# Luoyadan/CRB-active-3Ddet

Measured on AMD Instinct MI355X. Metric: frames/s SECOND fwd+bwd, KITTI 20k-pt clouds, higher is better.
Workload: dtype f32

## Files before the change

### crb-active-3ddet_amd/pcdet/models/backbones_2d/base_bev_backbone.py

```python
import numpy as np
import torch
import torch.nn as nn

from crbhip import bnrelu

from ...utils.fold_utils import fold_conv_bn
from ...utils.linear_rows import LinearRows, rows_view, rows_to_nchw


ROWS_TRAIN = True
ROWS_GEMM = True
WINOGRAD = __import__('os').environ.get('CRB_WINOGRAD', '1') != '0'


def _wino_fold(w, shift):
    from crbhip import winograd
    return winograd.weights_forward2(w), shift.contiguous()


def _wino_ok(conv, x, pad=None):
    if not WINOGRAD or not isinstance(conv, nn.Conv2d) or not x.is_cuda or x.dtype != torch.float32:
        return False
    from crbhip import winograd
    p = tuple(conv.padding) if pad is None else tuple(pad)
# ... 66 lines not shown
                if rows_ok:
                    y = m(x) if pad is None else torch.nn.functional.conv2d(x, m.weight, None, m.stride, pad, m.dilation,
                                                                             m.groups)
                    rows_ok = y.is_contiguous(memory_format=torch.channels_last) and \
                        bnrelu.supported(y.new_empty((2, y.shape[1])), bn)
                if rows_ok:
                    n, c, h, w_ = y.shape
                    rows = y.permute(0, 2, 3, 1).reshape(n * h * w_, c)
                    z = bnrelu.bn_apply_(rows, bn, relu)
                    x = z.view(n, h, w_, c).permute(0, 3, 1, 2)
                else:
                    w, shift = fold_conv_bn(m, bn)
                    if isinstance(m, nn.Conv2d):
                        x = torch.nn.functional.conv2d(x, w, shift, m.stride, m.padding if pad is None else pad, m.dilation,
                                                       m.groups)
                    else:
                        x = torch.nn.functional.conv_transpose2d(x, w, shift, m.stride, m.padding, m.output_padding,
                                                                 m.groups, m.dilation)
                    if relu:
                        x = torch.relu_(x)
                i += 3 if relu else 2
            else:
                x = m(x) if pad is None else torch.nn.functional.conv2d(x, m.weight, m.bias, m.stride, pad, m.dilation, m.groups)
                i += 1
        return x

    @staticmethod
    def _pad_conv(mods, i, x):
        m = mods[i]
        if isinstance(m, nn.ZeroPad2d) and i + 1 < len(mods) and isinstance(mods[i + 1], nn.Conv2d):
            c = mods[i + 1]
            pd = m.padding
            if c.padding == (0, 0) and c.padding_mode == 'zeros' and pd[0] == pd[1] and pd[2] == pd[3]:
                if _wino_ok(c, x, (pd[2], pd[0])):
                    from crbhip import winograd
                    return BaseBEVBackbone._wino_conv(c, x, mods[i + 2] if i + 2 < len(mods) else None), 2
                if torch.are_deterministic_algorithms_enabled() and torch.is_grad_enabled() and pd[0] == pd[2] and x.is_cuda:
                    from crbhip import dense_strided
                    if dense_strided.supported(c, x):
                        return dense_strided.conv_det(c, x, (pd[2], pd[0])), 2
                return torch.nn.functional.conv2d(x, c.weight, c.bias, c.stride, (pd[2], pd[0]), c.dilation, c.groups), 2
        return None, 0

    @staticmethod
    def _wino_conv(conv, x, nxt):
        from crbhip import winograd
        if winograd.STATS and conv.bias is None and isinstance(nxt, nn.BatchNorm2d) and nxt.training and \
                nxt.momentum is not None and bnrelu.FUSE_RUNNING and torch.is_grad_enabled() and not bnrelu.frame_groups_active():
            y, slabs = winograd.conv3x3_stats(x, conv.weight)
            y._crb_bn_slabs = slabs
            return y
        return winograd.conv3x3(x, conv.weight, conv.bias)

    @staticmethod
    def _run_rows_train(seq, x):
        mods = list(seq)
        i = 0
        while i < len(mods):
            m = mods[i]
            nxt = mods[i + 1] if i + 1 < len(mods) else None
            y, used = BaseBEVBackbone._pad_conv(mods, i, x)
            if used:
                x, i = y, i + used
                continue
            if _wino_ok(m, x):
                x = BaseBEVBackbone._wino_conv(m, x, nxt)
                i += 1
                continue
            if isinstance(m, nn.BatchNorm2d) and isinstance(nxt, nn.ReLU) and \
                    x.is_contiguous(memory_format=torch.channels_last) and \
                    bnrelu.supported(x.new_empty((2, x.shape[1])), m):
                n, c, h, w_ = x.shape
                rows = x.permute(0, 2, 3, 1).reshape(n * h * w_, c)
                slabs = getattr(x, '_crb_bn_slabs', None)
                x = bnrelu.bn_relu(rows, m, relu=True, slabs=slabs).view(n, h, w_, c).permute(0, 3, 1, 2)
                i += 2
            else:
                x = m(x)
                i += 1
        return x

    @staticmethod
    def _up(conv, x):
        if ROWS_GEMM and x.is_cuda and conv.bias is None and conv.kernel_size == (1, 1) and conv.stride == (1, 1) and \
                conv.padding == (0, 0) and conv.groups == 1 and conv.dilation == (1, 1):
            rows = rows_view(x)
            if rows is not None:
                w2d = conv.weight[:, :, 0, 0]
                w2d = w2d.t() if isinstance(conv, nn.ConvTranspose2d) else w2d
                n, _, h, w_ = x.shape
                return rows_to_nchw(LinearRows.apply(rows, w2d), n, h, w_)
        if torch.are_deterministic_algorithms_enabled() and torch.is_grad_enabled() and x.is_cuda and isinstance(conv, nn.ConvTranspose2d):
            from crbhip import dense_strided
            if dense_strided.supported(conv, x):
                return dense_strided.conv_det(conv, x)
        return conv(x)

    def _can_fuse_concat_eval(self, x):
        if len(self.deblocks) != len(self.blocks) or len(self.deblocks) < 2:
            return False
        for d in self.deblocks:
            m = list(d)
            if len(m) != 3 or not isinstance(m[1], nn.BatchNorm2d) or not isinstance(m[2], nn.ReLU) or m[0].bias is not None \
                    or not bnrelu.supported(x.new_empty((2, m[1].num_features)), m[1]):
                return False
        return True

    def _can_fuse_concat(self, x):
        if not self.training or len(self.deblocks) != len(self.blocks) or len(self.deblocks) < 2:
            return False
        for d in self.deblocks:
            m = list(d)
            if len(m) != 3 or not isinstance(m[1], nn.BatchNorm2d) or not isinstance(m[2], nn.ReLU) or \
                    not m[1].training or m[1].momentum is None or \
                    not bnrelu.supported(x.new_empty((2, m[1].num_features)), m[1]):
                return False
        return x.is_contiguous(memory_format=torch.channels_last)

    def forward(self, data_dict):
        spatial_features = data_dict['spatial_features']
        ups = []
        x = spatial_features
        if not self.training and not torch.is_grad_enabled():
            cat_ok = x.is_cuda and x.is_contiguous(memory_format=torch.channels_last) and self._can_fuse_concat_eval(x)
            pre = []
            for i, blk in enumerate(self.blocks):
                x = self._run_folded(blk, x)
                if cat_ok:
                    pre.append(self._up(self.deblocks[i][0], x))
                else:
                    ups.append(self._run_folded(self.deblocks[i], x) if len(self.deblocks) > 0 else x)
            if cat_ok and all(p.is_contiguous(memory_format=torch.channels_last) and p.shape[2:] == pre[0].shape[2:]
                              for p in pre):
                n, _, h, w_ = pre[0].shape
                cat = torch.empty((n * h * w_, sum(p.shape[1] for p in pre)), dtype=torch.float32, device=x.device)
                col = 0
                for d, p in zip(self.deblocks, pre):
                    bnrelu.bn_apply_into(p.permute(0, 2, 3, 1).reshape(n * h * w_, p.shape[1]), d[1], True, cat, col)
                    col += p.shape[1]
                ups = [cat.view(n, h, w_, cat.shape[1]).permute(0, 3, 1, 2)]
            elif cat_ok:
                ups = [self._run_folded(nn.Sequential(*list(d)[1:]), p) for d, p in zip(self.deblocks, pre)]
            x = torch.cat(ups, dim=1) if len(ups) > 1 else ups[0]
            if len(self.deblocks) > len(self.blocks):
                x = self._run_folded(self.deblocks[-1], x)
            data_dict['spatial_features_2d'] = x
            return data_dict
        run = self._run_rows_train if (ROWS_TRAIN and x.is_cuda and x.is_contiguous(memory_format=torch.channels_last)) \
            else (lambda seq, t: seq(t))
        if run == self._run_rows_train and torch.is_grad_enabled():
            from crbhip import winograd
            if winograd.PREPARE:
                winograd.prepare_weights2([m.weight for blk in self.blocks for m in blk
                                           if isinstance(m, nn.Conv2d) and m.kernel_size == (3, 3) and m.stride == (1, 1)
                                           and m.weight.is_cuda])
        fuse_cat = ROWS_TRAIN and x.is_cuda and self._can_fuse_concat(x)
        pre = []
        for i, blk in enumerate(self.blocks):
            x = run(blk, x)
            stride = int(spatial_features.shape[2] / x.shape[2])
            data_dict['spatial_features_%dx' % stride] = x
            if fuse_cat:
                pre.append(self._up(self.deblocks[i][0], x))
            else:
                ups.append(run(self.deblocks[i], x) if len(self.deblocks) > 0 else x)
        if fuse_cat and all(p.is_contiguous(memory_format=torch.channels_last) and p.shape[2:] == pre[0].shape[2:]
# ... 16 lines not shown
```

### include/crb_hip.h

```cpp
#ifndef CRB_HIP_H
#define CRB_HIP_H
#include <stdint.h>

#ifdef __cplusplus
extern "C" {
#endif

#define CRB_OK 0
#define CRB_ERR_ARG (-1)
#define CRB_ERR_WORKSPACE (-2)
#define CRB_ERR_LAUNCH (-3)
#define CRB_ERR_UNSUPPORTED (-4)

int crb_abi_version(void);

int64_t crb_voxelize_workspace_bytes(int64_t n_points, int B, int max_voxels, int max_points);
int crb_voxelize(const float* points, int64_t n_points, int num_features,
                 const int32_t* frame_offsets, int B,
                 const float* range_min_xyz, const float* voxel_size_xyz, const int32_t* grid_xyz,
                 int max_voxels, int max_points,
                 float* voxels, int32_t* coords, int32_t* num_points, float* mean_features,
                 int32_t* num_voxels_out,
                 void* workspace, int64_t workspace_bytes, void* stream);

// ... 308 lines not shown
                         float loss_weight, float* loss, float* d_preds, void* stream);
int crb_point_focal_loss_per_frame(const float* preds, const int64_t* labels, int64_t n, int num_class, int B, float alpha, float gamma,
                                   float loss_weight, float* loss, float* d_preds, void* stream);

typedef struct CrbRcnnLossCfg {
  float beta;
  float code_weights[7];
  float cls_weight, reg_weight, corner_weight;
  int32_t corner;
} CrbRcnnLossCfg;
int crb_rcnn_loss(const float* rcnn_cls, const float* rcnn_reg, const void* cls_labels, int labels_are_int64,
                  const int64_t* reg_valid_mask, const float* rois, const float* gt_of_rois, const float* gt_of_rois_src,
                  int gt_row_stride, int64_t n, const CrbRcnnLossCfg* cfg, float* loss, float* d_cls, float* d_reg,
                  float* reg_targets, void* stream);
int crb_rcnn_loss_per_frame(const float* rcnn_cls, const float* rcnn_reg, const void* cls_labels, int labels_are_int64,
                            const int64_t* reg_valid_mask, const float* rois, const float* gt_of_rois, const float* gt_of_rois_src,
                            int gt_row_stride, int64_t n, int B, const CrbRcnnLossCfg* cfg, float* loss_frames, float* d_cls, float* d_reg,
                            float* reg_targets, void* stream);
int crb_scale_rows_per_frame(const float* src, int64_t rows, int width, int frames, const float* g, float* dst, void* stream);
int crb_roi_canonical_targets(const float* rois, int roi_row_stride, const float* gt_of_rois, int gt_row_stride, int64_t n,
                              float* out, void* stream);
int crb_roi_grid_points(const float* rois, int roi_row_stride, int64_t n, int grid_size, float* out, void* stream);
int crb_rcnn_decode_boxes(const float* rois, int roi_row_stride, const float* box_preds, int64_t n, float* out, void* stream);
int crb_record_rows(const int64_t* sel, const uint8_t* valid, const float* box_preds, int box_row_stride, const float* cls_confs,
                    const int64_t* label_preds, const float* full_cls_scores, int full_classes, int B, int N, int P, int num_class,
                    float* pred_boxes, float* pred_scores, int64_t* pred_labels, float* pred_logits, float* entropy, void* stream);
int crb_box_point_density(const int32_t* first_box, const float* pred_boxes, int box_row_stride, const uint8_t* valid, int B, int M, int P,
                          float* density, void* stream);
typedef struct CrbRoiSamplerCfg {
  int32_t roi_per_image;
  int32_t fg_quota;
  int32_t by_class;
  int32_t score_type;
  float fg_thresh;
  float reg_fg_thresh, cls_fg_thresh, cls_bg_thresh, cls_bg_thresh_lo, hard_bg_ratio;
  float soft_den;
} CrbRoiSamplerCfg;
int crb_roi_sample_targets(const float* rois, int roi_row_stride, const float* roi_scores, const int64_t* roi_labels,
                           const float* gt_boxes, int gt_row_stride, const float* iou, const float* u_perm, const float* u_slot,
                           int B, int R, int G, const CrbRoiSamplerCfg* cfg, int64_t* sampled, float* out_rois, float* out_gt,
                           float* out_iou, float* out_scores, int64_t* out_labels, int64_t* reg_valid_mask, void* cls_labels,
                           void* stream);

int crb_winograd2_supported(int cin, int cout, int H, int W);
int64_t crb_winograd2_weights_bytes(int cin, int cout);
int crb_winograd2_weights(const float* g, float* U, int cin, int cout, void* stream);
int crb_winograd2_weights_conv(const float* w, int64_t so, int64_t si, int64_t sky, int64_t skx, float* U, int conv_cin,
                               int conv_cout, int mode, void* stream);
int crb_winograd2_weights_conv_multi(int n, const float* const* w, const int64_t* strides, float* const* U, const int32_t* conv_cin,
                                     const int32_t* conv_cout, const int32_t* mode, void* stream);
int crb_conv3x3_winograd2_nhwc(const float* x, const float* U, float* y, int N, int H, int W, int cin, int cout,
                               const float* bias, int relu, void* stream);
int64_t crb_winograd2_stats_slabs(int N, int H, int W);
int crb_conv3x3_winograd2_stats_nhwc(const float* x, const float* U, float* y, float* stats, int N, int H, int W, int cin, int cout,
                                     void* stream);

int crb_winograd4_supported(int cin, int cout, int H, int W);
int64_t crb_winograd4_weights_bytes(int cin, int cout);
int crb_winograd4_weights_conv(const float* w, int64_t so, int64_t si, int64_t sky, int64_t skx, void* U, int conv_cin, int conv_cout,
                               int mode, void* stream);
int crb_winograd4_weights_conv_multi(int n, const float* const* w, const int64_t* strides, void* const* U, const int32_t* conv_cin,
                                     const int32_t* conv_cout, const int32_t* mode, void* stream);
int crb_conv3x3_winograd4_nhwc(const float* x, const void* U, float* y, int N, int H, int W, int cin, int cout, const float* bias,
                               int relu, void* stream);
int64_t crb_winograd4_stats_slabs(int N, int H, int W);
int crb_conv3x3_winograd4_stats_nhwc(const float* x, const void* U, float* y, float* stats, int N, int H, int W, int cin, int cout,
                                     void* stream);
int crb_winograd4c_supported(int cin, int cout, int H, int W);
int crb_conv3x3_winograd4c_nhwc(const float* x, const void* U, float* y, int N, int H, int W, int cin, int cout,
                                const float* bias, int relu, void* stream);
int64_t crb_winograd4c_stats_slabs(int N, int H, int W);
int crb_conv3x3_winograd4c_stats_nhwc(const float* x, const void* U, float* y, float* stats, int N, int H, int W, int cin,
                                      int cout, void* stream);

int crb_winograd2_wgrad_supported(int cin, int cout, int H, int W);
int64_t crb_winograd2_wgrad_workspace_bytes(int cin, int cout);
int crb_winograd2_wgrad(const float* x, const float* dy, float* dw, int64_t so, int64_t si, int64_t sky, int64_t skx,
                        int N, int H, int W, int cin, int cout, void* workspace, int64_t workspace_bytes, void* stream);
int crb_winograd4_wgrad_supported(int cin, int cout, int H, int W);
int64_t crb_winograd4_wgrad_workspace_bytes(int cin, int cout);
int crb_winograd4_wgrad(const float* x, const float* dy, float* dw, int64_t so, int64_t si, int64_t sky, int64_t skx,
                        int N, int H, int W, int cin, int cout, void* workspace, int64_t workspace_bytes, void* stream);

int crb_cu_reservation(int cus, void* stream);

int crb_bev_interpolate_forward(const float* bev, int B, int H, int W, int C, const float* keypoints, int64_t M, float x_min,
                                float y_min, float voxel_x, float voxel_y, float bev_stride, float* out, void* stream);
int crb_bev_interpolate_backward(const float* dout, int B, int H, int W, int C, const float* keypoints, int64_t M, float x_min,
                                 float y_min, float voxel_x, float voxel_y, float bev_stride, float* dbev, void* stream);

#define CRB_LOSSNET_MAX_LAYERS 4
typedef struct CrbLossNetArgs {
  const float* x[CRB_LOSSNET_MAX_LAYERS];
  const float* w[CRB_LOSSNET_MAX_LAYERS];
  const float* gamma[CRB_LOSSNET_MAX_LAYERS];
  const float* beta[CRB_LOSSNET_MAX_LAYERS];
  float* running_mean[CRB_LOSSNET_MAX_LAYERS];
  float* running_var[CRB_LOSSNET_MAX_LAYERS];
  int64_t* num_batches_tracked[CRB_LOSSNET_MAX_LAYERS];
  int32_t channels[CRB_LOSSNET_MAX_LAYERS];
  int32_t num_layer;
  int32_t rows_per_frame;
  int32_t frames;
  int32_t training;
  float momentum, eps;
} CrbLossNetArgs;
typedef struct CrbLossNetGrads {
  float* d_x[CRB_LOSSNET_MAX_LAYERS];
  float* d_w[CRB_LOSSNET_MAX_LAYERS];
  float* d_gamma_beta;
  float* d_lin_w;
  float* d_lin_b;
} CrbLossNetGrads;
int64_t crb_lossnet_workspace_bytes(int num_layer, int64_t rows);
int crb_lossnet_forward(const CrbLossNetArgs* args, const float* lin_w, const float* lin_b, float* out, void* ws, int64_t ws_bytes,
                        void* stream);
int crb_lossnet_backward(const CrbLossNetArgs* args, const float* lin_w, const float* d_out, void* ws, int64_t ws_bytes,
                         const CrbLossNetGrads* grads, void* stream);

#ifdef __cplusplus
}
#endif
#endif
```

Baseline: 464.7.

## Add split-bf16 MFMA row GEMM kernels for BEV upsampling deconvolutions

Adds a custom HIP kernel family that runs the BEV backbone's kernel-equals-stride transposed convolutions (and 1x1 convs) as row GEMMs on bf16 MFMA. Each f32 operand is split into three bf16 parts to keep f32-level accuracy. The kernels cover forward, input-gradient and weight-gradient, with cached pre-swizzled weight images and a partial-sum reduction for wgrad. By default they are enabled for the stride-1 input-grad and the stride-2 forward, input-grad and wgrad launches. The aim is to replace vendor conv_transpose/GEMM calls with fused tiled kernels, at the cost of more MFMA passes per product and a weight-image rebuild whenever the weights change.

```diff
diff --git a/crb-active-3ddet_amd/crbhip/rows_gemm.py b/crb-active-3ddet_amd/crbhip/rows_gemm.py
--- /dev/null
+++ b/crb-active-3ddet_amd/crbhip/rows_gemm.py
@@ -0,0 +1,220 @@
+import os
+
+import numpy as np
+import torch
+
+from ._lib import lib, check, ptr, cur_stream, require_cuda, CrbHipError
+
+KERNEL = os.environ.get('CRB_ROWS_GEMM_KERNEL', 'x6')
+DEFAULT_LAUNCHES = '1i,2f,2i,2w'
+LAUNCHES = set(v.strip() for v in os.environ.get('CRB_ROWS_GEMM_LAUNCHES', DEFAULT_LAUNCHES).split(',') if v.strip())
+FORWARD, INPUT_GRAD, WGRAD = 0, 1, 2
+_DIR = 'fiw'
+
+
+def supported(cin, cout, stride, direction):
+    return bool(lib.crb_rows_gemm4_supported(int(cin), int(cout), int(stride), int(direction)))
+
+
+def use(cin, cout, stride, direction):
+    return KERNEL == 'x6' and ('%d%s' % (stride, _DIR[direction])) in LAUNCHES and supported(cin, cout, stride, direction)
+
+
+def _geometry(conv):
+    import torch.nn as nn
+    if not isinstance(conv, (nn.Conv2d, nn.ConvTranspose2d)) or conv.bias is not None or conv.groups != 1:
+        return None
+    if conv.dilation != (1, 1) or conv.padding != (0, 0) or getattr(conv, 'padding_mode', 'zeros') != 'zeros':
+        return None
+    k, s = conv.kernel_size, conv.stride
+    if k[0] != k[1] or s[0] != s[1] or k[0] != s[0] or s[0] not in (1, 2):
+        return None
+    transposed = isinstance(conv, nn.ConvTranspose2d)
+    if transposed and conv.output_padding != (0, 0):
+        return None
+    if not transposed and s[0] != 1:
+        return None
+    return conv.in_channels, conv.out_channels, s[0], transposed
+
+
+def dispatch(conv, x):
+    g = _geometry(conv)
+    if KERNEL != 'x6':
+        return 'vendor', 'CRB_ROWS_GEMM_KERNEL=%s' % KERNEL
+    if g is None:
+        return 'vendor', 'not a bias-free kernel = stride convolution with stride 1 or 2'
+    if not (x.is_cuda and x.dim() == 4 and x.dtype == torch.float32 and x.is_contiguous(memory_format=torch.channels_last)):
+        return 'vendor', 'input is not an f32 channels_last device map'
+    cin, cout, s, _ = g
+    on = [d for d in range(3) if use(cin, cout, s, d)]
+    if not on:
+        return 'vendor', 'no launch of %d -> %d stride %d is switched on with an instance' % (cin, cout, s)
+    return 'x6', ''.join(_DIR[d] for d in on)
+
+
+def _strides(weight, transposed):
+    st = weight.stride()
+    return (st[0], st[1], st[2], st[3]) if transposed else (st[1], st[0], st[2], st[3])
+
+
+_IMAGES = {}
+
+
+def weights(weight, cin, cout, stride, direction, transposed=True):
+    require_cuda(weight)
+    w = weight.detach()
+    key = (w.data_ptr(), w.device.index, int(direction))
+    tag = (w._version, tuple(w.shape), tuple(w.stride()), cin, cout, stride, transposed)
+    hit = _IMAGES.get(key)
+    if hit is not None and hit[0] == tag:
+        return hit[1]
+    if w.dtype != torch.float32:
+        raise CrbHipError('crb_rows_gemm4_weights takes f32 weights')
+    img = torch.empty((int(lib.crb_rows_gemm4_weights_bytes(cin, cout, stride)),), dtype=torch.uint8, device=w.device)
+    s_ci, s_co, s_a, s_b = _strides(w, transposed)
+    check(lib.crb_rows_gemm4_weights(w.data_ptr(), s_ci, s_co, s_a, s_b, ptr(img), cin, cout, stride, int(direction),
+                                     cur_stream(w.device)), 'crb_rows_gemm4_weights')
+    if len(_IMAGES) > 64:
+        _IMAGES.clear()
+    _IMAGES[key] = (tag, img, w)
+    return img
+
+
+def weight_image_reference(w, stride, direction):
+    w = np.asarray(w, dtype=np.float32)
+    cin, cout, s = w.shape[0], w.shape[1], int(stride)
+    T = s * s
+    wm = w.reshape(cin, cout, T).transpose(0, 2, 1).reshape(cin, T * cout)
+    if direction == INPUT_GRAD:
+        wm = wm.T
+    K, N = wm.shape
+    ks, lane, j = np.meshgrid(np.arange(K // 16), np.arange(64), np.arange(8), indexing='ij')
+    k = 32 * (ks >> 1) + 16 * (lane >> 5) + 8 * (ks & 1) + j
+    r = lane & 31
+    out = np.empty((N // 32, K // 16, 3, 64, 8), dtype=np.uint16)
+    for nb in range(N // 32):
+        v = np.ascontiguousarray(wm[k, 32 * nb + r])
+        for p in range(3):
+            hi = v.view(np.uint32) & np.uint32(0xffff0000)
+            out[nb, :, p] = (hi >> np.uint32(16)).astype(np.uint16)
+            v = v - hi.view(np.float32)
+    return out
+
+
+def _nhwc(x):
+    if not x.is_contiguous(memory_format=torch.channels_last):
+        x = x.contiguous(memory_format=torch.channels_last)
+    return x.permute(0, 2, 3, 1)
+
+
+def forward_x6(x, weight, cin, cout, s, transposed=True):
+    require_cuda(x, weight)
+    xv = _nhwc(x)
+    N, H, W, _ = xv.shape
+    img = weights(weight, cin, cout, s, FORWARD, transposed)
+    y = torch.empty((N, cout, s * H, s * W), dtype=torch.float32, device=x.device, memory_format=torch.channels_last)
+    check(lib.crb_rows_gemm4_forward(xv.data_ptr(), ptr(img), y.data_ptr(), N, H, W, cin, cout, s, cur_stream(x.device)),
+          'crb_rows_gemm4_forward')
+    return y
+
+
+def input_grad_x6(dy, weight, cin, cout, s, transposed=True):
+    require_cuda(dy, weight)
+    gv = _nhwc(dy)
+    N, Hs, Ws, _ = gv.shape
+    H, W = Hs // s, Ws // s
+    img = weights(weight, cin, cout, s, INPUT_GRAD, transposed)
+    dx = torch.empty((N, cin, H, W), dtype=torch.float32, device=dy.device, memory_format=torch.channels_last)
+    check(lib.crb_rows_gemm4_input_grad(gv.data_ptr(), ptr(img), dx.data_ptr(), N, H, W, cin, cout, s, cur_stream(dy.device)),
+          'crb_rows_gemm4_input_grad')
+    return dx
+
+
+_WGRAD_WS = {}
+
+
+def wgrad_x6(x, dy, like, cin, cout, s, transposed=True):
+    require_cuda(x, dy)
+    xv, gv = _nhwc(x), _nhwc(dy)
+    N, H, W, _ = xv.shape
+    if tuple(gv.shape) != (N, s * H, s * W, cout):
+        raise CrbHipError('rows_gemm wgrad: dy does not belong to x')
+    dw = torch.empty_like(like, dtype=torch.float32)
+    nbytes = int(lib.crb_rows_gemm4_wgrad_workspace_bytes(cin, cout, s))
+    key = (x.device, torch.cuda.current_stream(x.device).cuda_stream)
+    ws = _WGRAD_WS.get(key)
+    if ws is None or ws.numel() * 4 < nbytes:
+        ws = _WGRAD_WS[key] = torch.empty((nbytes // 4,), dtype=torch.float32, device=x.device)
+    s_ci, s_co, s_a, s_b = _strides(dw, transposed)
+    check(lib.crb_rows_gemm4_wgrad(xv.data_ptr(), gv.data_ptr(), dw.data_ptr(), s_ci, s_co, s_a, s_b, N, H, W, cin, cout, s, ptr(ws),
+                                   ws.numel() * 4, cur_stream(x.device)), 'crb_rows_gemm4_wgrad')
+    return dw
+
+
+def _vendor_forward(x, weight, s, transposed):
+    if s == 1:
+        from pcdet.utils.linear_rows import rows_view, rows_to_nchw
+        w2d = weight[:, :, 0, 0]
+        w2d = w2d.t() if transposed else w2d
+        n, _, h, w_ = x.shape
+        return rows_to_nchw(rows_view(x) @ w2d.t(), n, h, w_)
+    return torch.nn.functional.conv_transpose2d(x, weight, None, s, 0)
+
+
+class _UpConv(torch.autograd.Function):
+
+    @staticmethod
+    def forward(ctx, x, weight, cin, cout, s, transposed, det_wgrad=False):
+        ctx.save_for_backward(x, weight)
+        ctx.geo = (cin, cout, s, transposed)
+        ctx.det_wgrad = det_wgrad
+        if use(cin, cout, s, FORWARD):
+            return forward_x6(x, weight, cin, cout, s, transposed)
+        return _vendor_forward(x, weight, s, transposed)
+
+    @staticmethod
+    def backward(ctx, dy):
+        x, weight = ctx.saved_tensors
+        cin, cout, s, transposed = ctx.geo
+        dy = dy.contiguous(memory_format=torch.channels_last)
+        dx = dw = None
+        if ctx.needs_input_grad[0]:
+            if use(cin, cout, s, INPUT_GRAD):
+                dx = input_grad_x6(dy, weight, cin, cout, s, transposed)
+            elif s == 1:
+                from pcdet.utils.linear_rows import rows_view, rows_to_nchw
+                w2d = weight[:, :, 0, 0]
+                w2d = w2d.t() if transposed else w2d
+                n, _, h, w_ = x.shape
+                dx = rows_to_nchw(rows_view(dy) @ w2d, n, h, w_)
+            else:
+                dx = torch.ops.aten.convolution_backward(dy, x, weight, None, [s, s], [0, 0], [1, 1], True, [0, 0], 1,
+                                                         [True, False, False])[0]
+        if ctx.needs_input_grad[1]:
+            if ctx.det_wgrad:
+                from . import dense_strided
+                dw = dense_strided.weight_grad('deconv', x, dy, s, s, s, 0)
+            elif use(cin, cout, s, WGRAD):
+                dw = wgrad_x6(x, dy, weight, cin, cout, s, transposed)
+            elif s == 1:
+                from pcdet.utils.linear_rows import rows_view, tall_t_matmul
+                d2 = tall_t_matmul(rows_view(dy), rows_view(x))
+                dw = (d2.t() if transposed else d2).reshape(weight.shape)
+            else:
+                dw = torch.ops.aten.convolution_backward(dy, x, weight, None, [s, s], [0, 0], [1, 1], True, [0, 0], 1,
+                                                         [False, True, False])[1]
+        return dx, dw, None, None, None, None, None
+
+
+def up_conv(conv, x):
+    path, _ = dispatch(conv, x)
+    if path != 'x6':
+        return None
+    cin, cout, s, transposed = _geometry(conv)
+    det_wgrad = False
+    if s != 1 and torch.are_deterministic_algorithms_enabled() and torch.is_grad_enabled():
+        from . import dense_strided
+        if not (use(cin, cout, s, FORWARD) and use(cin, cout, s, INPUT_GRAD) and transposed and dense_strided.supported(conv, x)):
+            return None
+        det_wgrad = True
+    return _UpConv.apply(x, conv.weight, cin, cout, s, transposed, det_wgrad)
diff --git a/crb-active-3ddet_amd/csrc/rows_gemm4.hip b/crb-active-3ddet_amd/csrc/rows_gemm4.hip
--- /dev/null
+++ b/crb-active-3ddet_amd/csrc/rows_gemm4.hip
@@ -0,0 +1,538 @@
+#include <atomic>
+#include <type_traits>
+#include <utility>
+#include "crb_common.h"
+#include "winograd_split.h"
+#include "../../include/crb_hip.h"
+
+typedef float f32x4 __attribute__((ext_vector_type(4)));
+
+namespace {
+
+constexpr int NT = 256;
+
+template <typename F, int... I>
+__device__ __forceinline__ void static_for_impl(F&& f, std::integer_sequence<int, I...>) {
+  (f(std::integral_constant<int, I>{}), ...);
+}
+template <int N, typename F>
+__device__ __forceinline__ void static_for(F&& f) { static_for_impl(f, std::make_integer_sequence<int, N>{}); }
+
+template <int B>
+__device__ __forceinline__ void mfma_acc(const bf16x8& A, const bf16x8& Bv) {
+  asm volatile("v_mfma_f32_32x32x16_bf16 a[%2:%3], %0, %1, a[%2:%3]" : : "v"(A), "v"(Bv), "n"(B * 16), "n"(B * 16 + 15));
+}
+template <int R>
+__device__ __forceinline__ float acc_read() {
+  float x;
+  asm volatile("v_accvgpr_read_b32 %0, a[%1]" : "=v"(x) : "n"(R));
+  return x;
+}
+template <int R>
+__device__ __forceinline__ void acc_zero() { asm volatile("v_accvgpr_write_b32 a[%0], 0" : : "n"(R)); }
+__device__ __forceinline__ void acc_settle() { asm volatile("s_nop 15\n\ts_nop 15" ::: "memory"); }
+
+#define RG_ACC_0_127                                                                                                                   \
+  "a0", "a1", "a2", "a3", "a4", "a5", "a6", "a7", "a8", "a9", "a10", "a11", "a12", "a13", "a14", "a15", "a16", "a17", "a18", "a19",   \
+      "a20", "a21", "a22", "a23", "a24", "a25", "a26", "a27", "a28", "a29", "a30", "a31", "a32", "a33", "a34", "a35", "a36", "a37",   \
+      "a38", "a39", "a40", "a41", "a42", "a43", "a44", "a45", "a46", "a47", "a48", "a49", "a50", "a51", "a52", "a53", "a54", "a55",   \
+      "a56", "a57", "a58", "a59", "a60", "a61", "a62", "a63", "a64", "a65", "a66", "a67", "a68", "a69", "a70", "a71", "a72", "a73",   \
+      "a74", "a75", "a76", "a77", "a78", "a79", "a80", "a81", "a82", "a83", "a84", "a85", "a86", "a87", "a88", "a89", "a90", "a91",   \
+      "a92", "a93", "a94", "a95", "a96", "a97", "a98", "a99", "a100", "a101", "a102", "a103", "a104", "a105", "a106", "a107", "a108", \
+      "a109", "a110", "a111", "a112", "a113", "a114", "a115", "a116", "a117", "a118", "a119", "a120", "a121", "a122", "a123", "a124", \
+      "a125", "a126", "a127"
+#define RG_ACC_128_255                                                                                                                 \
+  "a128", "a129", "a130", "a131", "a132", "a133", "a134", "a135", "a136", "a137", "a138", "a139", "a140", "a141", "a142", "a143",     \
+      "a144", "a145", "a146", "a147", "a148", "a149", "a150", "a151", "a152", "a153", "a154", "a155", "a156", "a157", "a158", "a159", \
+      "a160", "a161", "a162", "a163", "a164", "a165", "a166", "a167", "a168", "a169", "a170", "a171", "a172", "a173", "a174", "a175", \
+      "a176", "a177", "a178", "a179", "a180", "a181", "a182", "a183", "a184", "a185", "a186", "a187", "a188", "a189", "a190", "a191", \
+      "a192", "a193", "a194", "a195", "a196", "a197", "a198", "a199", "a200", "a201", "a202", "a203", "a204", "a205", "a206", "a207", \
+      "a208", "a209", "a210", "a211", "a212", "a213", "a214", "a215", "a216", "a217", "a218", "a219", "a220", "a221", "a222", "a223", \
+      "a224", "a225", "a226", "a227", "a228", "a229", "a230", "a231", "a232", "a233", "a234", "a235", "a236", "a237", "a238", "a239", \
+      "a240", "a241", "a242", "a243", "a244", "a245", "a246", "a247", "a248", "a249", "a250", "a251", "a252", "a253", "a254", "a255"
+
+__device__ constexpr int pass_a(int p) { return p == 0 ? 0 : p == 1 ? 2 : p == 2 ? 1 : p == 3 ? 0 : p == 4 ? 1 : 0; }
+__device__ constexpr int pass_b(int p) { return p == 0 ? 2 : p == 1 ? 0 : p == 2 ? 1 : p == 3 ? 1 : 0; }
+
+struct Split8 {
+  float sv[2], s1[2], s2[2];
+  u32x4 q0, q1, q2;
+  template <int E>
+  __device__ __forceinline__ void put(float v) {
+    constexpr int hh = E & 1;
+    sv[hh] = v;
+    split3f(v, s1[hh], s2[hh]);
+    if constexpr (hh == 1) {
+      q0[E >> 1] = __builtin_amdgcn_perm(__float_as_uint(sv[1]), __float_as_uint(sv[0]), 0x07060302u);
+      q1[E >> 1] = __builtin_amdgcn_perm(__float_as_uint(s1[1]), __float_as_uint(s1[0]), 0x07060302u);
+      q2[E >> 1] = __builtin_amdgcn_perm(__float_as_uint(s2[1]), __float_as_uint(s2[0]), 0x07060302u);
+    }
+  }
+  __device__ __forceinline__ void get(bf16x8 (&f)[3]) const {
+    f[0] = __builtin_bit_cast(bf16x8, q0);
+    f[1] = __builtin_bit_cast(bf16x8, q1);
+    f[2] = __builtin_bit_cast(bf16x8, q2);
+  }
+};
+
+__global__ __launch_bounds__(256) void rows_gemm4_weights_kernel(const float* __restrict__ w, int64_t s_ci, int64_t s_co, int64_t s_a,
+                                                                 int64_t s_b, unsigned char* __restrict__ img, int cin, int cout, int s,
+                                                                 int direction, int K, int N) {
+  const int KS = K >> 4;
+  const int64_t id = (int64_t)blockIdx.x * 256 + threadIdx.x;
+  if (id >= (int64_t)(N >> 5) * KS * 64) return;
+  const int lane = (int)(id & 63), r = lane & 31, h = lane >> 5;
+  const int ks = (int)((id >> 6) % KS), nb = (int)((id >> 6) / KS);
+  const int n = nb * 32 + r, k0 = (ks >> 1) * 32 + h * 16 + (ks & 1) * 8;
+  u32x4 q[3];
+  unsigned lo[3] = {0, 0, 0};
+#pragma unroll
+  for (int j = 0; j < 8; ++j) {
+    const int k = k0 + j;
+    const int ci = direction ? n : k, tc = direction ? k : n;
+    const int t = tc / cout, co = tc - t * cout;
+    const float v = w[ci * s_ci + co * s_co + (t / s) * s_a + (t % s) * s_b];
+    unsigned p[3];
+    split3(v, p[0], p[1], p[2]);
+#pragma unroll
+    for (int i = 0; i < 3; ++i) {
+      if (j & 1) q[i][j >> 1] = lo[i] | (p[i] << 16);
+      else lo[i] = p[i];
+    }
+  }
+  unsigned char* dst = img + ((int64_t)(nb * KS + ks) * 3) * 1024 + lane * 16;
+#pragma unroll
+  for (int i = 0; i < 3; ++i) *reinterpret_cast<u32x4*>(dst + i * 1024) = q[i];
+}
+
+constexpr int RG_LDS_BYTES = 4 * 32 * 64 * 16;
+
+struct RgArgs {
+  const float* x;
+  float* y;
+  const unsigned char* wimg;
+  int M;
+  int W, s;
+  int kseg, nseg;
+  int tin, tout;
+  int K, N;
+  int ldx, ldy;
+  int wrn;
+  int col_tiles, tiles;
+};
+
+__device__ __forceinline__ unsigned big_pix(int m, int W, int s) { return (unsigned)(s * (m + (s - 1) * W * (m / W))); }
+
+__global__ __launch_bounds__(NT, 1) void rows_gemm4_kernel(RgArgs a) {
+  extern __shared__ __attribute__((aligned(16))) unsigned char rg_lds[];
+  asm volatile("" ::: RG_ACC_0_127, RG_ACC_128_255);
+  const int lane = threadIdx.x & 63, wave = __builtin_amdgcn_readfirstlane(threadIdx.x >> 6);
+  const int wr = wave % a.wrn, wc = wave / a.wrn, r = lane & 31, h = lane >> 5;
+  const int tile_rows = a.wrn * 64, tile_cols = (4 / a.wrn) * 128;
+  const int KC = a.K >> 5, KS = a.K >> 4, kcs = a.kseg >> 5;
+  int lt = blockIdx.x, lc = 0;
+  if (lt >= a.tiles) return;
+  const unsigned char* const wl = a.wimg + lane * 16;
+  const int Ws = a.W * a.s;
+
+  static_for<256>([](auto rc) { acc_zero<decltype(rc)::value>(); });
+
+  unsigned xpix[2];
+  auto set_xpix = [&](int tile) __attribute__((always_inline)) {
+#pragma unroll
+    for (int rb = 0; rb < 2; ++rb) {
+      const int m = min((tile / a.col_tiles) * tile_rows + wr * 64 + rb * 32 + r, a.M - 1);
+      xpix[rb] = a.tin > 1 ? big_pix(m, a.W, a.s) : (unsigned)m;
+    }
+  };
+  auto load_a = [&](int c, f32x4 (&dst)[2][4]) __attribute__((always_inline)) {
+    const int t = c / kcs, cs = c - t * kcs;
+    const unsigned tap = a.tin > 1 ? (unsigned)((t / a.s) * Ws + (t % a.s)) : 0u;
+#pragma unroll
+    for (int rb = 0; rb < 2; ++rb) {
+      const float* p = a.x + (size_t)(xpix[rb] + tap) * a.ldx + cs * 32 + h * 16;
+#pragma unroll
+      for (int q = 0; q < 4; ++q) dst[rb][q] = *reinterpret_cast<const f32x4*>(p + 4 * q);
+    }
+  };
+  auto load_b = [&](int tile, int ks, bf16x8 (&dst)[4][3]) __attribute__((always_inline)) {
+    const int nb0 = ((tile % a.col_tiles) * tile_cols + wc * 128) >> 5;
+#pragma unroll
+    for (int cb = 0; cb < 4; ++cb)
+#pragma unroll
+      for (int p = 0; p < 3; ++p)
+        dst[cb][p] = *reinterpret_cast<const bf16x8*>(wl + ((size_t)((nb0 + cb) * KS + ks) * 3 + p) * 1024);
+  };
+  auto step = [&](const bf16x8 (&Bw)[4][3], const bf16x8 (&Xf)[2][3], auto&& gap) __attribute__((always_inline)) {
+    static_for<48>([&](auto kc) __attribute__((always_inline)) {
+      constexpr int k = decltype(kc)::value, cb = k / 12, rb = (k / 6) & 1, pass = k % 6;
+      mfma_acc<(pass == 5 ? 0 : 8) + 4 * rb + cb>(Bw[cb][pass_a(pass)], Xf[rb][pass_b(pass)]);
+      gap(kc);
+      __builtin_amdgcn_sched_barrier(0);
+    });
+  };
+
+  f32x4 Ahi[2][2];
+  bf16x8 XF0[2][3], B0[4][3];
+  set_xpix(lt);
+  {
+    f32x4 A0[2][4];
+    load_a(0, A0);
+    load_b(lt, 0, B0);
+#pragma unroll
+    for (int rb = 0; rb < 2; ++rb) {
+      Split8 sp;
+      static_for<8>([&](auto ec) { constexpr int e = decltype(ec)::value; sp.put<e>(A0[rb][e >> 2][e & 3]); });
+      sp.get(XF0[rb]);
+      Ahi[rb][0] = A0[rb][2];
+      Ahi[rb][1] = A0[rb][3];
+    }
+  }
+  asm volatile("s_nop 4" ::: "memory");
+
+  for (;;) {
+    int nt = lt, nc = lc + 1;
+    if (nc == KC) { nc = 0; nt = lt + (int)gridDim.x; }
+    const bool more = nt < a.tiles;
+    if (!more) { nt = lt; nc = lc; }
+    bf16x8 B1[4][3];
+    load_b(lt, 2 * lc + 1, B1);
+    if (nt != lt) set_xpix(nt);
+    f32x4 An[2][4];
+    load_a(nc, An);
+    __builtin_amdgcn_sched_barrier(0);
+
+    bf16x8 XF1[2][3];
+    Split8 sp;
+    step(B0, XF0, [&](auto kc) __attribute__((always_inline)) {
+      constexpr int k = decltype(kc)::value;
+      if constexpr (k < 16) {
+        constexpr int rb = k >> 3, e = k & 7;
+        sp.put<e>(Ahi[rb][e >> 2][e & 3]);
+        if constexpr (e == 7) sp.get(XF1[rb]);
+      }
+    });
+    bf16x8 B0n[4][3];
+    load_b(nt, 2 * nc, B0n);
+    __builtin_amdgcn_sched_barrier(0);
+    bf16x8 XF0n[2][3];
+    step(B1, XF1, [&](auto kc) __attribute__((always_inline)) {
+      constexpr int k = decltype(kc)::value;
+      if constexpr (k >= 24 && k < 40) {
+        constexpr int rb = (k - 24) >> 3, e = (k - 24) & 7;
+        sp.put<e>(An[rb][e >> 2][e & 3]);
+        if constexpr (e == 7) sp.get(XF0n[rb]);
+      }
+    });
+
+    if (a.tin > 1 && lc != KC - 1 && (lc + 1) % kcs == 0) {
+      f32x4* const part = reinterpret_cast<f32x4*>(rg_lds) + wave * (32 * 64) + lane;
+      const bool first = lc + 1 == kcs;
+      acc_settle();
+      static_for<32>([&](auto qc) __attribute__((always_inline)) {
+        constexpr int R0 = 4 * decltype(qc)::value;
+        f32x4 v = (f32x4){acc_read<R0>(), acc_read<R0 + 1>(), acc_read<R0 + 2>(), acc_read<R0 + 3>()};
+        if (!first) v += part[decltype(qc)::value * 64];
+        part[decltype(qc)::value * 64] = v;
+      });
+      static_for<128>([](auto rc) { acc_zero<decltype(rc)::value>(); });
+      asm volatile("s_nop 4" ::: "memory");
+    }
+    if (lc == KC - 1) {
+      const int ctile = lt % a.col_tiles;
+      const int col0 = ctile * tile_cols + wc * 128;
+      const int tseg = col0 / a.nseg, ncol = col0 - tseg * a.nseg;
+      const unsigned tap = a.tout > 1 ? (unsigned)((tseg / a.s) * Ws + (tseg % a.s)) : 0u;
+      acc_settle();
+      static_for<2>([&](auto rbc) __attribute__((always_inline)) {
+        constexpr int rb = decltype(rbc)::value;
+        const int m = (lt / a.col_tiles) * tile_rows + wr * 64 + rb * 32 + r;
+        const bool ok = m < a.M;
+        const unsigned pix = (a.tout > 1 ? big_pix(min(m, a.M - 1), a.W, a.s) : (unsigned)m) + tap;
+        float* const out = a.y + (size_t)pix * a.ldy + ncol + 4 * h;
+        static_for<16>([&](auto qc) __attribute__((always_inline)) {
+          constexpr int cb = decltype(qc)::value >> 2, j = decltype(qc)::value & 3, R0 = (4 * rb + cb) * 16 + 4 * j;
+          f32x4 v = (f32x4){acc_read<R0>() + acc_read<128 + R0>(), acc_read<R0 + 1>() + acc_read<129 + R0>(),
+                            acc_read<R0 + 2>() + acc_read<130 + R0>(), acc_read<R0 + 3>() + acc_read<131 + R0>()};
+          if (a.tin > 1) v += (reinterpret_cast<const f32x4*>(rg_lds) + wave * (32 * 64) + lane)[(R0 / 4) * 64];
+          if (ok) *reinterpret_cast<f32x4*>(out + cb * 32 + 8 * j) = v;
+        });
+      });
+      static_for<256>([](auto rc) { acc_zero<decltype(rc)::value>(); });
+      asm volatile("s_nop 4" ::: "memory");
+    }
+    if (!more) break;
+#pragma unroll
+    for (int rb = 0; rb < 2; ++rb) {
+      Ahi[rb][0] = An[rb][2];
+      Ahi[rb][1] = An[rb][3];
+#pragma unroll
+      for (int p = 0; p < 3; ++p) XF0[rb][p] = XF0n[rb][p];
+    }
+#pragma unroll
+    for (int cb = 0; cb < 4; ++cb)
+#pragma unroll
+      for (int p = 0; p < 3; ++p) B0[cb][p] = B0n[cb][p];
+    lt = nt;
+    lc = nc;
+  }
+}
+
+constexpr int WCB = 256;
+constexpr int WIMG_G = WCB * 16;
+constexpr int WIMG_P = 2 * WIMG_G;
+constexpr int WIMG_OP = 3 * WIMG_P;
+constexpr int WIMG_BUF = 2 * WIMG_OP;
+constexpr int WLDS_BYTES = 2 * WIMG_BUF;
+
+struct RwArgs {
+  const float* x;
+  const float* dy;
+  float* part;
+  int M, W, s, T;
+  int cin, cout, nci, nco;
+  int nchunks;
+  int nranges;
+};
+
+__global__ __launch_bounds__(NT, 1) void rows_gemm4_wgrad_kernel(RwArgs a) {
+  extern __shared__ __attribute__((aligned(16))) unsigned char lds[];
+  asm volatile("" ::: RG_ACC_0_127, RG_ACC_128_255);
+  const int c = threadIdx.x, lane = c & 63, wave = __builtin_amdgcn_readfirstlane(c >> 6);
+  const int nb = a.T * a.nci * a.nco;
+  const int xcd = blockIdx.x & 7, slot = blockIdx.x >> 3;
+  const int sub = slot % nb, range = (slot / nb) * 8 + xcd;
+  if (range >= a.nranges) return;
+  const int t = sub % a.T, blk = sub / a.T;
+  const int cib = blk / a.nco, cob = blk - cib * a.nco;
+  const int c_first = (int)((int64_t)range * a.nchunks / a.nranges);
+  const int c_end = (int)((int64_t)(range + 1) * a.nchunks / a.nranges);
+  const int total = c_end - c_first;
+
+  static_for<256>([](auto rc) { acc_zero<decltype(rc)::value>(); });
+
+  const float* const xp = a.x + cib * WCB + c;
+  const float* const gp = a.dy + cob * WCB + c;
+  const unsigned tap = (unsigned)((t / a.s) * (a.W * a.s) + (t % a.s));
+  int xm = c_first * 16;
+  int gm = xm, gq = gm / a.W, gr = gm - gq * a.W;
+  float val[32];
+  unsigned gpix = tap;
+  auto request = [&](auto ic) __attribute__((always_inline)) {
+    constexpr int i = decltype(ic)::value;
+    if constexpr (i < 16) {
+      val[i] = xp[(size_t)min(xm, a.M - 1) * a.cin];
+      ++xm;
+    } else {
+      if (gm < a.M) gpix = (unsigned)(a.s * (gm + (a.s - 1) * a.W * gq)) + tap;
+      val[i] = gp[(size_t)gpix * a.cout];
+      ++gm;
+      if (++gr == a.W) { gr = 0; ++gq; }
+    }
+  };
+  Split8 sp;
+  auto value = [&](auto ic, unsigned char* buf, int m0) __attribute__((always_inline)) {
+    constexpr int i = decltype(ic)::value, e = i & 7, g = (i >> 3) & 1, op = i >> 4;
+    sp.put<e>(m0 + (i & 15) < a.M ? val[i] : 0.f);
+    if constexpr (e == 7) {
+      unsigned char* const dst = buf + op * WIMG_OP + g * WIMG_G + c * 16;
+      *reinterpret_cast<u32x4*>(dst) = sp.q0;
+      *reinterpret_cast<u32x4*>(dst + WIMG_P) = sp.q1;
+      *reinterpret_cast<u32x4*>(dst + 2 * WIMG_P) = sp.q2;
+    }
+  };
+
+  const int wi = wave & 1, wo = wave >> 1, l31 = lane & 31, lhi = lane >> 5;
+  const int a_rd = WIMG_OP + lhi * WIMG_G + (wo * 128 + l31) * 16;
+  const int b_rd = lhi * WIMG_G + (wi * 128 + l31) * 16;
+
+  if (total > 0) {
+    static_for<32>([&](auto ic) __attribute__((always_inline)) { request(ic); });
+    static_for<32>([&](auto ic) __attribute__((always_inline)) { value(ic, lds, c_first * 16); });
+    static_for<32>([&](auto ic) __attribute__((always_inline)) { request(ic); });
+    __syncthreads();
+    for (int q = 0; q < total; ++q) {
+      const unsigned char* const cur = lds + (q & 1) * WIMG_BUF;
+      unsigned char* const nxt = lds + ((q + 1) & 1) * WIMG_BUF;
+      bf16x8 A[4][3], B[4][3];
+#pragma unroll
+      for (int b = 0; b < 4; ++b)
+#pragma unroll
+        for (int p = 0; p < 3; ++p) {
+          if (b == 0) A[0][p] = *reinterpret_cast<const bf16x8*>(cur + a_rd + p * WIMG_P);
+          B[b][p] = *reinterpret_cast<const bf16x8*>(cur + b_rd + p * WIMG_P + b * 32 * 16);
+        }
+#pragma unroll
+      for (int b = 1; b < 4; ++b)
+#pragma unroll
+        for (int p = 0; p < 3; ++p) A[b][p] = *reinterpret_cast<const bf16x8*>(cur + a_rd + p * WIMG_P + b * 32 * 16);
+      __builtin_amdgcn_sched_barrier(0);
+      static_for<96>([&](auto kc) __attribute__((always_inline)) {
+        constexpr int k = decltype(kc)::value, bo = k / 24, bi = (k / 6) & 3, pass = k % 6;
+        mfma_acc<4 * bo + bi>(A[bo][pass_a(pass)], B[bi][pass_b(pass)]);
+        if constexpr ((k & 1) == 0 && k < 64) {
+          value(std::integral_constant<int, k / 2>{}, nxt, (c_first + q + 1) * 16);
+          request(std::integral_constant<int, k / 2>{});
+        }
+        __builtin_amdgcn_sched_barrier(0);
+      });
+      __syncthreads();
+    }
+  }
+
+  acc_settle();
+  float* const out = a.part + ((int64_t)range * nb + sub) * (WCB * WCB) + (wi * 128 + l31) * WCB + wo * 128 + 4 * lhi;
+  static_for<64>([&](auto qc) {
+    constexpr int Q = decltype(qc)::value, B = Q >> 2, j = Q & 3, bo = B >> 2, bi = B & 3;
+    const f32x4 v = (f32x4){acc_read<B * 16 + 4 * j>(), acc_read<B * 16 + 4 * j + 1>(), acc_read<B * 16 + 4 * j + 2>(),
+                            acc_read<B * 16 + 4 * j + 3>()};
+    *reinterpret_cast<f32x4*>(out + bi * 32 * WCB + bo * 32 + 8 * j) = v;
+  });
+}
+
+__global__ __launch_bounds__(256) void rows_gemm4_wgrad_reduce_kernel(const float* __restrict__ part, int nranges, int T, int nci, int nco,
+                                                                      int s, float* __restrict__ dw, int64_t s_ci, int64_t s_co,
+                                                                      int64_t s_a, int64_t s_b) {
+  const int sub = blockIdx.x / WCB, cil = blockIdx.x - sub * WCB, col = threadIdx.x;
+  const int t = sub % T, blk = sub / T, cib = blk / nco, cob = blk - cib * nco;
+  const int64_t nb = (int64_t)T * nci * nco;
+  const float* p = part + (int64_t)sub * (WCB * WCB) + cil * WCB + col;
+  double sum = 0.0;
+#pragma unroll 8
+  for (int r = 0; r < nranges; ++r) sum += (double)p[r * nb * (WCB * WCB)];
+  dw[(int64_t)(cib * WCB + cil) * s_ci + (int64_t)(cob * WCB + col) * s_co + (t / s) * s_a + (t % s) * s_b] = (float)sum;
+}
+
+__host__ int rg_cu_count() {
+  static std::atomic<int> n_cu{0};
+  int n = n_cu.load(std::memory_order_relaxed);
+  if (!n) {
+    int dev = 0;
+    hipDeviceProp_t prop;
+    if (hipGetDevice(&dev) != hipSuccess || hipGetDeviceProperties(&prop, dev) != hipSuccess) return 256;
+    n = prop.multiProcessorCount > 0 ? prop.multiProcessorCount : 256;
+    n_cu.store(n, std::memory_order_relaxed);
+  }
+  return n;
+}
+
+__host__ int rg_wgrad_ranges(int nb) {
+  const int r = (2 * rg_cu_count() / nb) & ~7;
+  return r < 8 ? 8 : r;
+}
+
+__host__ bool rg_shape_ok(int cin, int cout, int stride) {
+  return cin > 0 && cout > 0 && (stride == 1 || stride == 2) && cin <= 4096 && cout <= 4096;
+}
+
+__host__ int rg_launch(const float* x, const void* img, float* y, int64_t M, int W, int s, int kseg, int nseg, int tin, int tout,
+                       void* stream) {
+  RgArgs a;
+  a.x = x; a.y = y; a.wimg = (const unsigned char*)img;
+  a.M = (int)M; a.W = W; a.s = s;
+  a.kseg = kseg; a.nseg = nseg; a.tin = tin; a.tout = tout;
+  a.K = kseg * tin; a.N = nseg * tout;
+  a.ldx = kseg; a.ldy = nseg;
+  a.wrn = a.N % 256 == 0 ? 2 : 4;
+  const int tile_rows = a.wrn * 64, tile_cols = (4 / a.wrn) * 128;
+  a.col_tiles = a.N / tile_cols;
+  const int64_t tiles = ((M + tile_rows - 1) / tile_rows) * a.col_tiles;
+  if (tiles >= (1LL << 30)) return CRB_ERR_ARG;
+  a.tiles = (int)tiles;
+  const int grid = (int)(tiles < rg_cu_count() ? tiles : rg_cu_count());
+  static std::atomic<unsigned> attr_done[64];
+  int dev = 0;
+  CRB_HIP(hipGetDevice(&dev));
+  if (dev < 0 || dev >= 64) return CRB_ERR_ARG;
+  if (tin > 1 && !attr_done[dev].load(std::memory_order_acquire)) {
+    CRB_HIP(hipFuncSetAttribute((const void*)rows_gemm4_kernel, hipFuncAttributeMaxDynamicSharedMemorySize, RG_LDS_BYTES));
+    attr_done[dev].store(1u, std::memory_order_release);
+  }
+  hipLaunchKernelGGL(rows_gemm4_kernel, dim3((unsigned)grid), dim3(NT), tin > 1 ? RG_LDS_BYTES : 0, (hipStream_t)stream, a);
+  CRB_CHECK_LAUNCH();
+  return CRB_OK;
+}
+
+}
+
+extern "C" int crb_rows_gemm4_supported(int cin, int cout, int stride, int direction) {
+  if (!rg_shape_ok(cin, cout, stride)) return 0;
+  if (direction == 0) return (cin % 32 == 0 && cout % 128 == 0) ? 1 : 0;
+  if (direction == 1) return (cout % 32 == 0 && cin % 128 == 0) ? 1 : 0;
+  if (direction == 2) return (cin % WCB == 0 && cout % WCB == 0) ? 1 : 0;
+  return 0;
+}
+
+extern "C" int64_t crb_rows_gemm4_weights_bytes(int cin, int cout, int stride) {
+  if (!rg_shape_ok(cin, cout, stride)) return 0;
+  return (int64_t)stride * stride * cin * cout * 6;
+}
+
+extern "C" int crb_rows_gemm4_weights(const float* w, int64_t s_ci, int64_t s_co, int64_t s_a, int64_t s_b, void* image, int cin,
+                                      int cout, int stride, int direction, void* stream) {
+  if (direction != 0 && direction != 1) return CRB_ERR_ARG;
+  if (!crb_rows_gemm4_supported(cin, cout, stride, direction)) return CRB_ERR_UNSUPPORTED;
+  if (!w || !image) return CRB_ERR_ARG;
+  const int T = stride * stride;
+  const int K = direction ? T * cout : cin, N = direction ? cin : T * cout;
+  const int64_t threads = (int64_t)(N / 32) * (K / 16) * 64;
+  hipLaunchKernelGGL(rows_gemm4_weights_kernel, dim3((unsigned)((threads + 255) / 256)), dim3(256), 0, (hipStream_t)stream, w, s_ci, s_co,
+                     s_a, s_b, (unsigned char*)image, cin, cout, stride, direction, K, N);
+  CRB_CHECK_LAUNCH();
+  return CRB_OK;
+}
+
+extern "C" int crb_rows_gemm4_forward(const float* x, const void* image, float* y, int N, int H, int W, int cin, int cout, int stride,
+                                      void* stream) {
+  if (N <= 0 || H <= 0 || W <= 0 || !x || !image || !y) return CRB_ERR_ARG;
+  if (!crb_rows_gemm4_supported(cin, cout, stride, 0)) return CRB_ERR_UNSUPPORTED;
+  const int64_t M = (int64_t)N * H * W, T = stride * stride;
+  if (M * T * (cin > cout ? cin : cout) >= (1LL << 31)) return CRB_ERR_ARG;
+  return rg_launch(x, image, y, M, W, stride, cin, cout, 1, (int)T, stream);
+}
+
+extern "C" int crb_rows_gemm4_input_grad(const float* dy, const void* image, float* dx, int N, int H, int W, int cin, int cout,
+                                         int stride, void* stream) {
+  if (N <= 0 || H <= 0 || W <= 0 || !dy || !image || !dx) return CRB_ERR_ARG;
+  if (!crb_rows_gemm4_supported(cin, cout, stride, 1)) return CRB_ERR_UNSUPPORTED;
+  const int64_t M = (int64_t)N * H * W, T = stride * stride;
+  if (M * T * (cin > cout ? cin : cout) >= (1LL << 31)) return CRB_ERR_ARG;
+  return rg_launch(dy, image, dx, M, W, stride, cout, cin, (int)T, 1, stream);
+}
+
+extern "C" int64_t crb_rows_gemm4_wgrad_workspace_bytes(int cin, int cout, int stride) {
+  if (!crb_rows_gemm4_supported(cin, cout, stride, 2)) return 0;
+  const int nb = stride * stride * (cin / WCB) * (cout / WCB);
+  return (int64_t)rg_wgrad_ranges(nb) * nb * WCB * WCB * 4;
+}
+
+extern "C" int crb_rows_gemm4_wgrad(const float* x, const float* dy, float* dw, int64_t s_ci, int64_t s_co, int64_t s_a, int64_t s_b,
+                                    int N, int H, int W, int cin, int cout, int stride, void* workspace, int64_t workspace_bytes,
+                                    void* stream) {
+  if (N <= 0 || H <= 0 || W <= 0 || !x || !dy || !dw) return CRB_ERR_ARG;
+  if (!crb_rows_gemm4_supported(cin, cout, stride, 2)) return CRB_ERR_UNSUPPORTED;
+  if (!workspace || workspace_bytes < crb_rows_gemm4_wgrad_workspace_bytes(cin, cout, stride)) return CRB_ERR_WORKSPACE;
+  const int64_t M = (int64_t)N * H * W, T = stride * stride;
+  if (M * T * (cin > cout ? cin : cout) >= (1LL << 31)) return CRB_ERR_ARG;
+  static std::atomic<unsigned> attr_done[64];
+  int dev = 0;
+  CRB_HIP(hipGetDevice(&dev));
+  if (dev < 0 || dev >= 64) return CRB_ERR_ARG;
+  if (!attr_done[dev].load(std::memory_order_acquire)) {
+    CRB_HIP(hipFuncSetAttribute((const void*)rows_gemm4_wgrad_kernel, hipFuncAttributeMaxDynamicSharedMemorySize, WLDS_BYTES));
+    attr_done[dev].store(1u, std::memory_order_release);
+  }
+  RwArgs a;
+  a.x = x; a.dy = dy; a.part = (float*)workspace;
+  a.M = (int)M; a.W = W; a.s = stride; a.T = (int)T;
+  a.cin = cin; a.cout = cout; a.nci = cin / WCB; a.nco = cout / WCB;
+  a.nchunks = (int)((M + 15) / 16);
+  const int nb = a.T * a.nci * a.nco;
+  a.nranges = rg_wgrad_ranges(nb);
+  hipLaunchKernelGGL(rows_gemm4_wgrad_kernel, dim3((unsigned)(a.nranges * nb)), dim3(NT), WLDS_BYTES, (hipStream_t)stream, a);
+  CRB_CHECK_LAUNCH();
+  hipLaunchKernelGGL(rows_gemm4_wgrad_reduce_kernel, dim3((unsigned)(nb * WCB)), dim3(256), 0, (hipStream_t)stream,
+                     (const float*)workspace, a.nranges, a.T, a.nci, a.nco, stride, dw, s_ci, s_co, s_a, s_b);
+  CRB_CHECK_LAUNCH();
+  return CRB_OK;
+}
diff --git a/crb-active-3ddet_amd/pcdet/models/backbones_2d/base_bev_backbone.py b/crb-active-3ddet_amd/pcdet/models/backbones_2d/base_bev_backbone.py
--- a/crb-active-3ddet_amd/pcdet/models/backbones_2d/base_bev_backbone.py
+++ b/crb-active-3ddet_amd/pcdet/models/backbones_2d/base_bev_backbone.py
@@ -172,6 +172,11 @@
 
     @staticmethod
     def _up(conv, x):
+        if ROWS_GEMM and x.is_cuda:
+            from crbhip import rows_gemm
+            y = rows_gemm.up_conv(conv, x)
+            if y is not None:
+                return y
         if ROWS_GEMM and x.is_cuda and conv.bias is None and conv.kernel_size == (1, 1) and conv.stride == (1, 1) and \
                 conv.padding == (0, 0) and conv.groups == 1 and conv.dilation == (1, 1):
             rows = rows_view(x)
diff --git a/include/crb_hip.h b/include/crb_hip.h
--- a/include/crb_hip.h
+++ b/include/crb_hip.h
@@ -414,6 +414,18 @@
 int crb_winograd4_wgrad(const float* x, const float* dy, float* dw, int64_t so, int64_t si, int64_t sky, int64_t skx,
                         int N, int H, int W, int cin, int cout, void* workspace, int64_t workspace_bytes, void* stream);
 
+int crb_rows_gemm4_supported(int cin, int cout, int stride, int direction);
+int64_t crb_rows_gemm4_weights_bytes(int cin, int cout, int stride);
+int crb_rows_gemm4_weights(const float* w, int64_t s_ci, int64_t s_co, int64_t s_a, int64_t s_b, void* image, int cin, int cout,
+                           int stride, int direction, void* stream);
+int crb_rows_gemm4_forward(const float* x, const void* image, float* y, int N, int H, int W, int cin, int cout, int stride,
+                           void* stream);
+int crb_rows_gemm4_input_grad(const float* dy, const void* image, float* dx, int N, int H, int W, int cin, int cout, int stride,
+                              void* stream);
+int64_t crb_rows_gemm4_wgrad_workspace_bytes(int cin, int cout, int stride);
+int crb_rows_gemm4_wgrad(const float* x, const float* dy, float* dw, int64_t s_ci, int64_t s_co, int64_t s_a, int64_t s_b, int N,
+                         int H, int W, int cin, int cout, int stride, void* workspace, int64_t workspace_bytes, void* stream);
+
 int crb_cu_reservation(int cus, void* stream);
 
 int crb_bev_interpolate_forward(const float* bev, int B, int H, int W, int C, const float* keypoints, int64_t M, float x_min,
```

After: 477.2, median of 6. 1.03x the previous value.
